# rsinghlab/GNN-Tumor-Seg

Hardware: AMD Instinct MI355X
Metric: supervoxel-graphs/sec training, 7xSAGE-pool-256, 15k-node graphs (higher is better)
Workload: dtype f32; 1 GPU; C2: 7xGraphSAGE-pool-256 (8 SAGEConv), fwd+weighted-CE+bwd+AdamW, 4 x 15000-node/86350-edge lattice graphs per GPU, 4-chan feat, fp32; global_batch=4, nodes_per_batch=60000, edges_per_batch=345400, parallelism=dp1

## Files before the change

### gnn-tumor-seg_amd/csrc/gts_gemm.hip

```cpp
#include "gts_gemm_tiles.h"
#include "gts_gemm_panel.h"
#include "gts_gemm_wgrad.h"
#include "gts_gemm_small.h"

namespace gts {
namespace {

template <bool AKC, bool BKC>
int pick_plain_variant(const GemmArgs& p) {
  int variant = BKC ? g_fwd_variant : g_igrad_variant;
  if (p.rb <= 128 && variant < 9) return 0;
  const bool row_count_invariant = variant == -2;
  if (variant < 0) {
    const int64_t cols = (p.rb + 255) / 256;
    const int64_t big_tiles = static_cast<int64_t>((p.ra + 255) / 256) * cols;
    variant = big_tiles >= 192 ? 8 : 3;
    if constexpr (AKC && BKC) {
      const int h = panel_rows_for(p.ra, cols);
      const int64_t panels = static_cast<int64_t>((p.ra + h - 1) / h) * cols;
      const int64_t rows256 = (big_tiles + 255) / 256 * 256, rows_panel = (panels + 255) / 256 * h;
      if (variant == 8 && rows_panel < rows256 && !row_count_invariant) variant = 10;
      if (variant == 3 && panels >= 192 && panels <= 256 && !row_count_invariant) variant = 10;
    }
  }
// ... 319 lines not shown
  r.splits = splits;
  int jobs = 0;
  for (int q = 0; q < n_problems; ++q, ++jobs) {
    r.slabs[jobs] = workspace + static_cast<size_t>(q) * splits * n * k;
    r.out[jobs] = gw[q], r.n4[jobs] = static_cast<int>(n * k / 4);
  }
  for (int q = 0; q < n_problems && any_bias; ++q) {
    if (!gb[q]) continue;
    r.slabs[jobs] = p.colsum + static_cast<size_t>(q) * splits * n;
    r.out[jobs] = gb[q], r.n4[jobs] = static_cast<int>(n / 4);
    ++jobs;
  }
  reduce_slabs_kernel<<<dim3(static_cast<unsigned>((n * k / 4 + 63) / 64), jobs), kBlock, 0, st>>>(r);
  return launch_status();
}
```

### gnn-tumor-seg_amd/csrc/gts_gemm_wgrad.h

```cpp
#pragma once
#include <type_traits>

#include "gts_gemm_tiles.h"

namespace gts {
namespace {

typedef float v2f __attribute__((ext_vector_type(2)));

template <int O0, int O1>
__device__ __forceinline__ v2f lds_read2st64(unsigned addr) {
  static_assert(O0 >= 0 && O1 <= 255, "ds_read2st64_b32 offsets are 8 bits");
  v2f r;
  asm volatile("ds_read2st64_b32 %0, %1 offset0:%2 offset1:%3" : "=v"(r) : "v"(addr), "n"(O0), "n"(O1));
  return r;
}

template <class Probe = NoProbe>
__global__ __launch_bounds__(1024, 4) void wgrad_stream_kernel(const GemmArgs p) {
  constexpr int BM = 256, BN = 256, WM = 4, WN = 4, WTM = 64, WTN = 64, TM = 2, TN = 2;
  constexpr int kPlane = kBK * BM;
  static_assert(BM == BN && kPlane * 4 == 128 * 256, "image I of an operand sits 128 offset units above image 0");
  __shared__ float lds[4 * kPlane];
  const int lane = threadIdx.x & 63, wave = __builtin_amdgcn_readfirstlane(threadIdx.x >> 6);
// ... 158 lines not shown
#pragma unroll 8
    for (int s = grp; s < p.splits; s += 4) acc += src[static_cast<size_t>(s) * n4];
  }
  part[grp][col] = acc;
  __syncthreads();
  if (grp == 0 && i < n4) {
    const v4f total = (part[0][col] + part[1][col]) + (part[2][col] + part[3][col]);
    reinterpret_cast<v4f*>(out)[i] = total;
  }
}

constexpr int kSkinnyMax = 9;
constexpr int kSkinnyChunks = 512;

template <int S>
__global__ __launch_bounds__(kBlock) void skinny_wgrad_kernel(const float* __restrict__ skinny, int s_cols,
                                                             const float* __restrict__ wide,
                                                             float* __restrict__ partial, int64_t m,
                                                             int w, int64_t rows_per_chunk) {
  __shared__ v4f red[kBlock];
  const int cols4 = w >> 2;
  const int lanes = cols4 >= kBlock ? 1 : kBlock / cols4;
  const int rl = cols4 >= kBlock ? 0 : threadIdx.x / cols4;
  const int64_t row0 = blockIdx.x * rows_per_chunk, row1 = min(m, row0 + rows_per_chunk);
  for (int q0 = 0; q0 < cols4; q0 += kBlock) {
    const int q = q0 + (cols4 >= kBlock ? threadIdx.x : threadIdx.x % cols4);
    const bool live = q < cols4 && rl < lanes;
    v4f acc[S];
#pragma unroll
    for (int i = 0; i < S; ++i) acc[i] = v4f{0.f, 0.f, 0.f, 0.f};
    if (live) {
#pragma unroll 4
      for (int64_t row = row0 + rl; row < row1; row += lanes) {
        const v4f f = *reinterpret_cast<const v4f*>(wide + static_cast<size_t>(row) * w + 4 * q);
#pragma unroll
// ... 3 lines not shown
#pragma unroll
    for (int i = 0; i < S; ++i) {
      v4f total = acc[i];
      if (lanes > 1) {
        __syncthreads();
        red[threadIdx.x] = acc[i];
        __syncthreads();
        if (rl == 0 && live) {
          for (int l = 1; l < lanes; ++l) total += red[l * cols4 + q];
        }
      }
      if (rl == 0 && live)
        *reinterpret_cast<v4f*>(partial + (static_cast<size_t>(blockIdx.x) * S + i) * w + 4 * q) = total;
    }
  }
}

__global__ __launch_bounds__(kBlock) void skinny_sum_kernel(const float* __restrict__ partial,
                                                           float* __restrict__ dst0,
                                                           float* __restrict__ dst1, int rows, int s_cols,
                                                           int w, int chunks, int transposed) {
  __shared__ float part[16][16];
  const int o = threadIdx.x & 15, lane = threadIdx.x >> 4;
  const int idx = blockIdx.x * 16 + o;
  const int total_out = rows * w;
  float acc = 0.f;
  if (idx < total_out) {
#pragma unroll 8
    for (int c = lane; c < chunks; c += 16) acc += partial[static_cast<size_t>(c) * total_out + idx];
  }
  part[lane][o] = acc;
  __syncthreads();
  if (lane != 0 || idx >= total_out) return;
  float sum = part[0][o];
#pragma unroll
  for (int l = 1; l < 16; ++l) sum += part[l][o];
  const int i = idx / w, j = idx - i * w;
  if (i < s_cols)
    dst0[transposed ? j * s_cols + i : i * w + j] = sum;
  else if (dst1 != nullptr)
    dst1[j] = sum;
}

inline int64_t skinny_workspace_floats(int64_t m, int64_t n, int64_t k) {
// ... 101 lines not shown
```

### gnn-tumor-seg_amd/csrc/gts_project.hip

```cpp
#include "gts_rows.h"

namespace gts {
namespace {

template <typename RowT>
__device__ __forceinline__ void store_row(RowT* dst, const RowT& v, int nt) {
  if (!nt) {
    *dst = v;
    return;
  }
  if constexpr (sizeof(RowT) == 16) {
    typedef unsigned u4 __attribute__((ext_vector_type(4)));
    __builtin_nontemporal_store(*reinterpret_cast<const u4*>(&v), reinterpret_cast<u4*>(dst));
  } else if constexpr (sizeof(RowT) == 8) {
    typedef unsigned u2 __attribute__((ext_vector_type(2)));
    __builtin_nontemporal_store(*reinterpret_cast<const u2*>(&v), reinterpret_cast<u2*>(dst));
  } else {
    __builtin_nontemporal_store(v, dst);
  }
}

constexpr int kVoxPerLane = 8;
constexpr int kVoxPerWave = kWave * kVoxPerLane;
constexpr int kVoxPerBlock = kVoxPerWave * kWavesPerBlock;
// ... 134 lines not shown
inline void launch_project_argmax(const int16_t* svs, const float* logits, const int16_t* relabel,
                                  int16_t* out, int64_t n_vox, int n_rows, int n_classes,
                                  uint8_t* occ, int dx, int dy, int dz, hipStream_t st) {
  const unsigned grid = stream_grid(n_vox);
  if (n_classes == 4 && (reinterpret_cast<uintptr_t>(logits) & 15) == 0)
    project_argmax_kernel<4><<<grid, kBlock, 0, st>>>(svs, logits, relabel, out, n_vox, n_rows, 4,
                                                      occ, dx, dy, dz);
  else
    project_argmax_kernel<0><<<grid, kBlock, 0, st>>>(svs, logits, relabel, out, n_vox, n_rows,
                                                      n_classes, occ, dx, dy, dz);
}

}
}

extern "C" int32_t gts_abi_version(void) { return 29; }

extern "C" const char* gts_error_string(int32_t code) {
  switch (code) {
    case GTS_OK: return "ok";
    case GTS_ERR_NULL: return "gts: required pointer is NULL";
    case GTS_ERR_SHAPE: return "gts: unsupported or inconsistent shape";
    case GTS_ERR_ARGKIND: return "gts: unsupported arg_bytes/row_bytes/mode";
    default: return code > 0 ? hipGetErrorString(static_cast<hipError_t>(code)) : "gts: unknown error";
  }
}

extern "C" int32_t gts_project_rows_i16(const int16_t* svs, const void* table,
                                        const void* bg_row, void* out, int64_t n_vox,
                                        int64_t n_rows, int32_t row_bytes, void* stream) {
  using namespace gts;
// ... 62 lines not shown
```

### gnn-tumor-seg_amd/csrc/gts_stack.hip

```cpp
#include <algorithm>
#include <vector>

#include "gts_gemm_args.h"

namespace {

constexpr int kMaxLayers = 64;

inline int64_t align256(int64_t bytes) { return (bytes + 255) & ~255LL; }

inline bool bad_stack(int64_t n_rows, const int64_t* widths, int32_t n_layers) {
  if (!widths || n_layers < 1 || n_layers > kMaxLayers || n_rows < 0 || n_rows >= (1LL << 31)) return true;
  for (int i = 0; i <= n_layers; ++i)
    if (widths[i] <= 0 || widths[i] % 4 != 0 || widths[i] >= (1 << 20)) return true;
  return false;
}

struct FwdPlan {
  int64_t m[kMaxLayers], arg[kMaxLayers], out[kMaxLayers], bits[kMaxLayers];
  int64_t p[2];
  int64_t wp[kMaxLayers][3];
  int64_t counters;
  int64_t total;
};
// ... 24 lines not shown
  p.total = at;
  return p;
}

inline bool chainable(int64_t n, int64_t k0, int64_t k1, int64_t n2) {
  return n % 4 == 0 && k0 % 4 == 0 && k1 % 4 == 0 && n <= 256 && n2 <= 256;
}

inline bool turns(int64_t rows, int64_t cols) { return cols >= 128 && rows % 4 == 0 && cols % 4 == 0; }

struct BwdPlan {
  int64_t wt[kMaxLayers][3];
  int64_t wtp[kMaxLayers][3];
  int64_t g[kMaxLayers], gp[kMaxLayers];
  int64_t gm[2];
  int64_t workspace, workspace_bytes;
  int64_t counters;
  int64_t total;
};

struct ByShape {
  struct Group {
    int64_t rows, cols;
    std::vector<const float*> in[2];
    std::vector<float*> out[2];
    int count() const { return static_cast<int>(in[0].size()); }
  };
  std::vector<Group> groups;
  void add(int64_t rows, int64_t cols, const float* in0, const float* in1, float* out0, float* out1) {
    auto it = std::find_if(groups.begin(), groups.end(), [&](const Group& c) { return c.rows == rows && c.cols == cols; });
// ... 6 lines not shown
inline int64_t weight_rows(const int64_t* w, int i, int q) { return q == 0 ? w[i] : w[i + 1]; }

inline BwdPlan plan_backward(int64_t n, const int64_t* w, int n_layers) {
  BwdPlan p{};
  int64_t at = 0, widest = 0;
  auto take = [&](int64_t bytes) { const int64_t o = at; at += align256(bytes); return o; };
  ByShape wgrads;
  for (int i = 0; i < n_layers; ++i) {
    const int64_t fin = w[i];
    widest = std::max(widest, fin);
    for (int q = 0; q < 3; ++q) p.wt[i][q] = turns(weight_rows(w, i, q), fin) ? take(4 * weight_rows(w, i, q) * fin) : -1;
    for (int q = 0; q < 3; ++q)
      p.wtp[i][q] = p.wt[i][q] >= 0 ? take(4 * gts_packed_weight_floats(fin, weight_rows(w, i, q))) : -1;
    p.g[i] = i > 0 ? take(4 * n * fin) : -1;
    p.gp[i] = take(4 * n * fin);
    for (int q = 0; q < 3; ++q) wgrads.add(weight_rows(w, i, q), fin, nullptr, nullptr, nullptr, nullptr);
  }
  p.gm[0] = take(4 * n * widest);
  p.gm[1] = take(4 * n * widest);
  int64_t ws = 0;
  if (n > 0)
    for (const auto& grp : wgrads.groups)
      for (int first = 0; first < grp.count(); first += gts::kMaxProblems)
        ws = std::max(ws, gts_linear_bwd_weight_workspace(n, grp.rows, grp.cols, std::min(gts::kMaxProblems, grp.count() - first)));
  p.workspace_bytes = ws;
  p.workspace = take(ws);
  p.counters = take(4 * GTS_CLUSTER_COUNTER_WORDS);
  p.total = at;
  return p;
}

// ... 150 lines not shown
  auto wt = [&](int i, int q) -> const float* { return plan.wt[i][q] >= 0 ? f32(plan.wt[i][q]) : nullptr; };
  auto wtp = [&](int i, int q) -> const float* { return plan.wtp[i][q] >= 0 ? f32(plan.wtp[i][q]) : nullptr; };

  auto igrad = [&](const float* g0, const float* w0, const float* w0t, int64_t n0, const float* g1, const float* w1,
                   const float* w1t, int64_t n1, const float* relu_mask, const uint64_t* relu_bits, float* gin,
                   int64_t k, const float* w0tp, const float* w1tp) -> int32_t {
    if (w0t != nullptr && (g1 == nullptr || w1t != nullptr)) {
      const float* packed[2] = {w0tp, g1 ? w1tp : nullptr};
      return gts_linear_bwd_input_t_f32(g0, w0t, g1, g1 ? w1t : nullptr, relu_mask, relu_mask ? relu_bits : nullptr, gin,
                                        n_rows, k, n0, g1 ? n1 : 0, packed, stream);
    }
    return gts_linear_bwd_input_f32(g0, w0, g1, g1 ? w1 : nullptr, relu_mask, gin, n_rows, k, n0, g1 ? n1 : 0, stream);
  };

  ByShape wgrads;

  const float* g = gout;
  const float* gm = nullptr;
  int cur = 0;
  for (int i = n_layers - 1; i >= 0; --i) {
    const float* w_pool = params[5 * i];
    const float* w_self = params[5 * i + 2];
    const float* w_neigh = params[5 * i + 3];
    const int64_t fin = widths[i], fout = widths[i + 1];
    const float* h = input_of(i);
    const float* m = act(fwd.m[i]);
    const void* arg = acts + fwd.arg[i];
    if (gm == nullptr) {
      float* buf = f32(plan.gm[cur]);
      GTS_TRY(igrad(g, w_neigh, wt(i, 2), fout, nullptr, nullptr, nullptr, 0, nullptr, nullptr, buf, fin, wtp(i, 2), nullptr));
      gm = buf;
    }
    float* gp = f32(plan.gp[i]);
    if (sched_rec != nullptr && fin == 256 && arg_bytes == 1 && n_rows * 1024 < (1LL << 32)) {
      GTS_TRY(gts_spmm_max_bwd_cluster_f32(sched_rec, sched_clusters, sched_rows, sched_srcs, sched_loc_words, gm, arg, 1, gp,
                                           n_rows, fin, counters, stream));
    } else {
      GTS_TRY(gts_spmm_max_bwd_f32(t_indptr, t_indices, t_slot, gm, arg, arg_bytes, nullptr, gp, n_rows, fin, stream));
    }
    gm = nullptr;
    wgrads.add(fin, fin, gp, h, grads[5 * i], grads[5 * i + 1]);
    wgrads.add(fout, fin, g, h, grads[5 * i + 2], grads[5 * i + 4]);
    wgrads.add(fout, fin, g, m, grads[5 * i + 3], nullptr);
    if (i > 0) {
      const int64_t below_in = widths[i - 1];
      const uint64_t* hbits = fwd.bits[i - 1] >= 0 ? reinterpret_cast<const uint64_t*>(acts + fwd.bits[i - 1]) : nullptr;
      float* g_next = f32(plan.g[i]);
      const float* below_t = wt(i - 1, 2);
      if (wt(i, 1) && wt(i, 0) && below_t && chainable(fin, fout, fin, below_in)) {
        float* gm_next = f32(plan.gm[cur ^ 1]);
        const float* packed[3] = {wtp(i, 1), wtp(i, 0), wtp(i - 1, 2)};
        GTS_TRY(gts_linear_bwd_input_chain_t_f32(g, wt(i, 1), gp, wt(i, 0), h, hbits, g_next, below_t, gm_next, n_rows, fin,
                                                 fout, fin, below_in, packed, stream));
        gm = gm_next, cur ^= 1;
      } else {
        GTS_TRY(igrad(g, w_self, wt(i, 1), fout, gp, w_pool, wt(i, 0), fin, h, hbits, g_next, fin, wtp(i, 1), wtp(i, 0)));
      }
      g = g_next;
    } else if (gx != nullptr) {
      GTS_TRY(igrad(g, w_self, wt(i, 1), fout, gp, w_pool, wt(i, 0), fin, nullptr, nullptr, gx, fin, wtp(i, 1), wtp(i, 0)));
    }
  }
  for (const auto& grp : wgrads.groups)
    for (int first = 0; first < grp.count(); first += gts::kMaxProblems)
      GTS_TRY(gts_linear_bwd_weight_f32(grp.in[0].data() + first, grp.in[1].data() + first, grp.out[0].data() + first,
                                        grp.out[1].data() + first, std::min(gts::kMaxProblems, grp.count() - first),
                                        f32(plan.workspace), plan.workspace_bytes, n_rows, grp.rows, grp.cols, stream));
  return GTS_OK;
}
```

### gnn-tumor-seg_amd/gts/_lib.py

```python
import ctypes
import os
import re

_HERE = os.path.dirname(os.path.abspath(__file__))
LIB_PATH = os.environ.get("GTS_LIB_PATH") or os.path.join(_HERE, "libgts_hip.so")
HEADER_PATH = os.path.join(os.path.dirname(os.path.dirname(_HERE)), "include", "gts_hip.h")
ABI_VERSION = 29

_p = ctypes.c_void_p
_i32 = ctypes.c_int32
_i64 = ctypes.c_int64
_f32 = ctypes.c_float
_f64 = ctypes.c_double

SIGNATURES = {
    "gts_abi_version": [],
    "gts_error_string": [_i32],
    "gts_spmm_max_fwd_f32": [_p, _p, _p, _p, _p, _i32, _i32, _i64, _i64, _p],
    "gts_spmm_max_bwd_f32": [_p, _p, _p, _p, _p, _i32, _p, _p, _i64, _i64, _p],
    "gts_cluster_record_words": [_i32, _i32, _i32, _i32],
    "gts_cluster_schedule": [_p, _p, _p, _p, _p, _i64, _i32, _i32, _i32, _p, _i64, _p, _p, _p],
    "gts_cluster_lds_bytes": [_i32, _i32, _i32, _i32],
    "gts_cluster_uses_counters": [_i64, _i32, _i32, _i32, _i32],
    "gts_spmm_max_fwd_cluster_f32": [_p, _i64, _i32, _i32, _i32, _p, _p, _p, _i32, _i32, _i64, _i64, _p, _p],
# ... 29 lines not shown
    "gts_relu_bits_bytes": [_i64, _i64],
    "gts_relu_bits_pay": [_i64, _i64],
    "gts_linear_bwd_input_f32": [_p, _p, _p, _p, _p, _p, _i64, _i64, _i64, _i64, _p],
    "gts_linear_bwd_input_t_f32": [_p, _p, _p, _p, _p, _p, _p, _i64, _i64, _i64, _i64, _p, _p],
    "gts_linear_bwd_input_t_act_workspace": [_i64, _i64],
    "gts_linear_bwd_input_t_act_f32": [_p, _p, _p, _p, _p, _i32, _p, _p, _p, _i64, _i64, _i64, _i64, _i64, _p, _p],
    "gts_transpose_batch_f32": [_p, _p, _i32, _i64, _i64, _p],
    "gts_packed_weight_floats": [_i64, _i64],
    "gts_pack_weights_f32": [_p, _p, _p, _i32, _i64, _i64, _i32, _p],
    "gts_gat_fc_scores_workspace": [_i64, _i64, _i64],
    "gts_gat_fc_scores_f32": [_p, _p, _p, _p, _p, _p, _p, _p, _i64, _i64, _i64, _i64, _i64, _p, _p],
    "gts_linear_fwd_chain_f32": [_p, _p, _p, _p, _p, _p, _p, _p, _p, _i64, _i64, _i64, _i64, _i32, _i64, _i32, _p, _p, _p],
    "gts_linear_bwd_input_chain_t_f32": [_p, _p, _p, _p, _p, _p, _p, _p, _p, _i64, _i64, _i64, _i64, _i64, _p, _p],
    "gts_linear_bwd_weight_workspace": [_i64, _i64, _i64, _i32],
    "gts_linear_bwd_weight_f32": [_p, _p, _p, _p, _i32, _p, _i64, _i64, _i64, _i64, _p],
    "gts_sage_pool_stack_fwd_arena": [_i64, _p, _i32, _i32, _i32, _i32, _p],
    "gts_sage_pool_stack_fwd_f32": [_p, _p, _p, _i64, _i32, _i32, _i32, _p, _p, _i64, _p, _i32, _i32, _i32, _i32, _p, _i64, _p],
    "gts_sage_pool_stack_bwd_scratch": [_i64, _p, _i32, _i32],
    "gts_sage_pool_stack_bwd_f32": [_p, _p, _p, _p, _i64, _i32, _i32, _i32, _p, _p, _p, _i64, _p, _i32, _i32, _i32, _p, _p, _p,
                                    _p, _i64, _p],
    "gts_set_option": [_i32, _i32],
    "gts_get_option": [_i32],
    "gts_weighted_ce_workspace": [_i64],
    "gts_weighted_ce_f32": [_p, _p, _p, _p, _p, _i64, _p, _i64, _i64, _p],
    "gts_dice_ce_workspace": [_i64, _i32],
    "gts_dice_ce_fwd_f32": [_p, _p, _p, _p, _i32, _f64, _f64, _f64, _p, _p, _i64, _i64, _i64, _p],
    "gts_dice_ce_bwd_f32": [_p, _p, _p, _p, _i32, _f64, _f64, _f64, _p, _p, _p, _i64, _i64, _p],
    "gts_collate_plan": [_p, _i32, _i64, _p, _i32, _p],
    "gts_collate_batch": [_p, _i32, _i64, _p, _i32, _p, _i64, _i32, _p],
    "gts_gg_gaussian_f64": [_p, _p, _p, _p, _i32, _f64, _i64, _i64, _i64, _i64, _p],
# ... 28 lines not shown
    "gts_intake_select_workspace": [],
    "gts_intake_order_stats": [_p, _i32, _i64, _i64, _i64, _p, _i64, _p, _i64, _p, _i64, _i64, _i64, _p, _p, _i64, _p],
    "gts_intake_standardize": [_p, _i32, _i64, _i64, _i64, _p, _i64, _p, _i64, _p, _i64, _p, _p, _p],
    "gts_dataset_stats_workspace": [_i64, _i64, _i64],
    "gts_dataset_stats_mask": [_p, _i32, _p, _i64, _i64, _i64, _p, _p, _i64, _p],
    "gts_dataset_stats_order_stats": [_p, _i32, _i64, _i64, _i64, _i64, _i64, _i64, _p, _p, _i64, _p],
    "gts_dataset_stats_moments": [_p, _i32, _i64, _i64, _i64, _i64, _p, _p, _p, _i64, _p],
    "gts_conform_gather": [_p, _i32, _i64, _i64, _i64, _i64, _i32, _i32, _i32, _i64, _i64, _i64, _p, _p, _p, _i32, _p, _p],
}
_RESTYPE = {"gts_error_string": ctypes.c_char_p, "gts_linear_bwd_weight_workspace": _i64,
            "gts_weighted_ce_workspace": _i64, "gts_gat_reduce_workspace": _i64,
            "gts_dice_ce_workspace": _i64,
            "gts_label_confusion_workspace": _i64, "gts_gat_fc_scores_workspace": _i64,
            "gts_relu_bits_bytes": _i64, "gts_cluster_record_words": _i64, "gts_sage_pool_stack_fwd_arena": _i64, "gts_sage_pool_stack_bwd_scratch": _i64, "gts_cluster_lds_bytes": _i64,
            "gts_linear_bwd_input_t_act_workspace": _i64, "gts_gat_cluster_workspace": _i64,
            "gts_packed_weight_floats": _i64, "gts_gg_sv_stats_workspace": _i64, "gts_gg_touching_workspace": _i64,
            "gts_conv3d_fwd_workspace": _i64, "gts_conv3d_bwd_data_workspace": _i64,
            "gts_conv3d_bwd_weight_workspace": _i64, "gts_hd95_workspace": _i64,
            "gts_intake_select_workspace": _i64, "gts_dataset_stats_workspace": _i64,
            "gts_components_workspace": _i64, "gts_lesionwise_workspace": _i64, "gts_lesionwise_table_ints": _i64}

COLLATE_MAX_SCHEDULES = 6


class CollateMember(ctypes.Structure):
    _fields_ = [("n_nodes", _i64), ("n_edges", _i64),
                ("indptr", _p), ("indices", _p), ("t_indptr", _p), ("t_indices", _p), ("t_slot", _p), ("t_pos", _p),
                ("features", _p), ("labels", _p), ("feat_bytes", _i32), ("label_bytes", _i32),
                ("sched_rec", _p * COLLATE_MAX_SCHEDULES), ("sched_clusters", _i64 * COLLATE_MAX_SCHEDULES),
                ("sched_loc_words", _i32 * COLLATE_MAX_SCHEDULES)]

# ... 80 lines not shown
```

### gnn-tumor-seg_amd/gts/dense.py

```python
import torch
import torch.nn.functional as F

from . import _lib
from ._lib import check, current_stream, ptr, require_device

GEMM_TIMER = None


class row_count_invariant:

    _depth = 0
    _saved = -1
    _lock = __import__("threading").Lock()

    def __enter__(self):
        with row_count_invariant._lock:
            if row_count_invariant._depth == 0:
                lib = _lib.load()
                row_count_invariant._saved = int(lib.gts_get_option(1))
                check(lib.gts_set_option(1, -2), "gts_set_option")
            row_count_invariant._depth += 1
        return self

    def __exit__(self, *exc):
# ... 342 lines not shown
                                          ptr(ws), ws.numel() * 4, m, n_p, k_p, current_stream()),
            "gts_linear_bwd_weight_f32"))
    out = []
    for gw, gb in zip(gws, gbs):
        if (n_p, k_p) != (n, k):
            gw = gw[:n, :k].contiguous()
            gb = gb[:n].contiguous() if gb is not None else None
        out.append((gw, gb))
    return out


def linear_bwd_weight(g, a, want_bias_grad=False):
    return linear_bwd_weight_multi([(g, a, want_bias_grad)])[0]


def relu_bwd(g, out):
    return g * (out > 0)


class _Linear(torch.autograd.Function):

    @staticmethod
    def forward(ctx, x, w, bias):
        ctx.save_for_backward(x, w)
        ctx.has_bias = bias is not None
        return linear_fwd(x, w, bias=bias)

    @staticmethod
    def backward(ctx, gy):
        x, w = ctx.saved_tensors
# ... 11 lines not shown
```

### gnn-tumor-seg_amd/gts/nn.py

```python
import os

import torch
import torch.nn as nn
import torch.nn.functional as F

from . import dense, ops


class GraphError(RuntimeError):
    """Counterpart of dgl.DGLError for the checks the layers make."""


def _is_relu(fn):
    return fn in (F.relu, torch.relu, torch.nn.functional.relu)


class _SagePoolLayer(torch.autograd.Function):

    @staticmethod
    def forward(ctx, g, h, w_pool, b_pool, w_self, w_neigh, bias, relu_out, need_bwd):
        h = h.contiguous()
        p = dense.linear_fwd(h, w_pool, bias=b_pool, relu=True)
        m, arg = ops.spmm_max_fwd(g, p, want_arg=need_bwd, relu_input=True)
        out = dense.linear_fwd(h, w_self, m, w_neigh, bias=bias, relu=relu_out)
# ... 163 lines not shown
        turned, turned_fragment = _pack_by_shape(
            [w for w in (params[5 * i + j] for i in range(n) for j in (0, 2, 3))
             if w.shape[1] >= 128 and w.shape[0] % 4 == 0 and w.shape[1] % 4 == 0], transposed=True, want_plain=True)

        def igrad(g0, w0, g1=None, w1=None, relu_mask=None, relu_bits=None):
            if id(w0) in turned and (w1 is None or id(w1) in turned) and g0.is_contiguous():
                return dense.linear_bwd_input_t(g0, turned[id(w0)], g1, turned[id(w1)] if w1 is not None else None,
                                                relu_mask=relu_mask, relu_bits=relu_bits,
                                                packed=(turned_fragment[id(w0)], turned_fragment[id(w1)] if w1 is not None else None))
            return dense.linear_bwd_input(g0, w0, g1, w1, relu_mask=relu_mask)

        def defer(grad_out, act, slot, bias_slot):
            key = (grad_out.shape[1], act.shape[1])
            deferred.setdefault(key, []).append((grad_out, act, bias_slot is not None, slot, bias_slot))

        gm = None
        for i in reversed(range(n)):
            h, m, arg, hbits = acts[4 * i:4 * i + 4]
            w_pool, _b_pool, w_self, w_neigh, _bias = params[5 * i:5 * i + 5]
            if gm is None:
                gm = igrad(g, w_neigh)
            gp = ops.spmm_max_bwd(ctx.g, gm, arg)
            gm = None
            defer(gp, h, 5 * i, 5 * i + 1)
            defer(g, h, 5 * i + 2, 5 * i + 4)
            defer(g, m, 5 * i + 3, None)
            if i > 0:
                below = params[5 * (i - 1) + 3]
                if all(id(w) in turned for w in (w_self, w_pool, below)) and _chainable(g, w_self.t(), gp, below.t()):
                    g, gm = dense.linear_bwd_input_chain_t(g, turned[id(w_self)], gp, turned[id(w_pool)], h,
                                                           turned[id(below)], relu_bits=hbits,
                                                           packed=(turned_fragment[id(w_self)], turned_fragment[id(w_pool)],
                                                                   turned_fragment[id(below)]))
                else:
                    g = igrad(g, w_self, gp, w_pool, relu_mask=h, relu_bits=hbits)
            elif ctx.needs_input_grad[1]:
                gx = igrad(g, w_self, gp, w_pool)
        for problems in deferred.values():
            results = dense.linear_bwd_weight_multi([(go, act, want) for go, act, want, _, _ in problems])
            for (gw, gb), (_, _, _, slot, bias_slot) in zip(results, problems):
                grads[slot] = gw
                if bias_slot is not None:
                    grads[bias_slot] = gb
        return (None, gx, None, *grads)


STACK_IN_ONE_CALL = os.environ.get("GTS_STACK_C", "1") != "0"


class GradSink:

    def __init__(self, params, extra=0):
        self.params = list(params)
        self.offsets, at = {}, 0
        for p in self.params:
            self.offsets[id(p)] = at
            at += p.numel()
        self.n, self.extra = at, int(extra)
# ... 394 lines not shown
```

### include/gts_hip.h

```cpp
#ifndef GTS_HIP_H
#define GTS_HIP_H

#include <stdint.h>

#ifdef __cplusplus
extern "C" {
#endif

#define GTS_OK 0
#define GTS_ERR_NULL (-1)
#define GTS_ERR_SHAPE (-2)
#define GTS_ERR_ARGKIND (-3)

int32_t gts_abi_version(void);
const char* gts_error_string(int32_t code);

int32_t gts_spmm_max_fwd_f32(const int32_t* indptr, const int32_t* indices, const float* x,
                             float* out, void* arg, int32_t arg_bytes, int32_t relu_input,
                             int64_t n_dst, int64_t n_feat, void* stream);

int32_t gts_spmm_max_bwd_f32(const int32_t* t_indptr, const int32_t* t_indices,
                             const int32_t* t_slot, const float* gout, const void* arg,
                             int32_t arg_bytes, const float* relu_src, float* gx,
                             int64_t n_src, int64_t n_feat, void* stream);
// ... 132 lines not shown
                                 float* out2, int64_t m, int64_t n, int64_t k0, int64_t k1, int32_t relu,
                                 int64_t n2, int32_t relu2, uint64_t* relu_bits, const float* const* packed,
                                 void* stream);
int32_t gts_linear_bwd_input_chain_t_f32(const float* g0, const float* w0t, const float* g1,
                                         const float* w1t, const float* relu_mask, const uint64_t* relu_bits,
                                         float* gin, const float* w2t, float* gin2, int64_t m, int64_t k,
                                         int64_t n0, int64_t n1, int64_t k2, const float* const* packed,
                                         void* stream);
int32_t gts_transpose_batch_f32(const float* const* src, float* const* dst, int32_t n_mats,
                                int64_t rows, int64_t cols, void* stream);
int64_t gts_linear_bwd_weight_workspace(int64_t m, int64_t n, int64_t k, int32_t n_problems);
int32_t gts_linear_bwd_weight_f32(const float* const* g, const float* const* a, float* const* gw,
                                  float* const* gb, int32_t n_problems, float* workspace,
                                  int64_t workspace_bytes, int64_t m, int64_t n, int64_t k,
                                  void* stream);

int64_t gts_sage_pool_stack_fwd_arena(int64_t n_rows, const int64_t* widths, int32_t n_layers, int32_t training,
                                      int32_t arg_bytes, int32_t relu_bits, int64_t* offsets);
int32_t gts_sage_pool_stack_fwd_f32(const int32_t* indptr, const int32_t* indices, const int32_t* sched_rec,
                                    int64_t sched_clusters, int32_t sched_rows, int32_t sched_srcs,
                                    int32_t sched_loc_words, const float* x, const float* const* params,
                                    int64_t n_rows, const int64_t* widths, int32_t n_layers, int32_t training,
                                    int32_t arg_bytes, int32_t relu_bits, void* arena, int64_t arena_bytes, void* stream);
int64_t gts_sage_pool_stack_bwd_scratch(int64_t n_rows, const int64_t* widths, int32_t n_layers, int32_t relu_bits);
int32_t gts_sage_pool_stack_bwd_f32(const int32_t* t_indptr, const int32_t* t_indices, const int32_t* t_slot,
                                    const int32_t* sched_rec, int64_t sched_clusters, int32_t sched_rows,
                                    int32_t sched_srcs, int32_t sched_loc_words, const float* gout, const float* x,
                                    const float* const* params, int64_t n_rows, const int64_t* widths,
                                    int32_t n_layers, int32_t arg_bytes, int32_t relu_bits, const void* fwd_arena,
                                    float* const* grads, float* gx, void* scratch, int64_t scratch_bytes,
// ... 176 lines not shown
```

Measured before the change: 955.8 graphs/s.

## Fuse narrow first/last SAGE layer backward into dedicated skinny kernels

Adds special backward paths for the narrow layers of the SAGE stack: the 4-channel input layer and the narrow output layer. For the first layer, one kernel fuses the input-gradient through w_neigh with the self/neigh weight-gradient partial sums and the bias sum. For the last layer, a skinny wgrad kernel also produces bias sums. Partials for all narrow layers are reduced at the end in a single batched sum-jobs kernel instead of going through the generic wide GEMM wgrad path. This cuts launches and wasted tile work on very skinny GEMMs, at the cost of extra workspace and more code paths.

```diff
diff --git a/gnn-tumor-seg_amd/csrc/gts_gemm.hip b/gnn-tumor-seg_amd/csrc/gts_gemm.hip
--- a/gnn-tumor-seg_amd/csrc/gts_gemm.hip
+++ b/gnn-tumor-seg_amd/csrc/gts_gemm.hip
@@ -357,3 +357,137 @@
   reduce_slabs_kernel<<<dim3(static_cast<unsigned>((n * k / 4 + 63) / 64), jobs), kBlock, 0, st>>>(r);
   return launch_status();
 }
+
+namespace gts {
+namespace {
+
+inline int narrow_kind(int64_t n, int64_t k) {
+  if (n <= 0 || k <= 0 || !aligned4(n) || !aligned4(k) || skinny_workspace_floats(1, n, k) == 0) return 0;
+  if (k < n) return (k == 4 || k == 8) && (n == 64 || n == 128 || n == 256) && g_igrad_variant <= 1 ? 1 : 0;
+  return n == 4 || n == 8 ? 2 : 0;
+}
+
+struct NarrowBlock {
+  int64_t first, second, sums, total;
+};
+inline NarrowBlock narrow_block(int kind, int64_t n, int64_t k) {
+  NarrowBlock b{};
+  if (kind == 1) b.second = kSkinnyChunks * (k + 1) * n, b.total = b.second + kSkinnyChunks * k * n;
+  if (kind == 2) b.second = kSkinnyChunks * n * k, b.sums = 2 * b.second, b.total = b.sums + kSkinnyChunks * n;
+  return b;
+}
+
+inline bool bad_narrow_rows(int64_t m) { return m < 0 || m >= (1LL << 31); }
+
+}
+}
+
+extern "C" int32_t gts_narrow_bwd_kind(int64_t n, int64_t k) { return gts::narrow_kind(n, k); }
+
+extern "C" int64_t gts_narrow_bwd_partial_floats(int64_t n, int64_t k) {
+  return gts::narrow_block(gts::narrow_kind(n, k), n, k).total;
+}
+
+extern "C" int32_t gts_narrow_bwd_first_f32(const float* g, const float* w_neigh, const float* x, const float* mact, float* gm,
+                                            float* partial, int32_t want_bias, int64_t m, int64_t n, int64_t k, void* stream) {
+  using namespace gts;
+  if (!g || !w_neigh || !x || !mact || !gm || !partial) return GTS_ERR_NULL;
+  if (bad_narrow_rows(m) || narrow_kind(n, k) != 1) return GTS_ERR_SHAPE;
+  if (m == 0) return GTS_OK;
+  hipStream_t st = static_cast<hipStream_t>(stream);
+  const NarrowBlock b = narrow_block(1, n, k);
+  const int64_t rpc = (m + kSkinnyChunks - 1) / kSkinnyChunks;
+  const int chunks = static_cast<int>((m + rpc - 1) / rpc), w = static_cast<int>(n);
+  float* px = partial;
+  float* pm = partial + b.second;
+  if (k == 4) {
+    if (want_bias) narrow_first_kernel<4, true><<<chunks, kBlock, 0, st>>>(g, w_neigh, x, mact, gm, px, pm, m, w, rpc);
+    else narrow_first_kernel<4, false><<<chunks, kBlock, 0, st>>>(g, w_neigh, x, mact, gm, px, pm, m, w, rpc);
+  } else {
+    if (want_bias) narrow_first_kernel<8, true><<<chunks, kBlock, 0, st>>>(g, w_neigh, x, mact, gm, px, pm, m, w, rpc);
+    else narrow_first_kernel<8, false><<<chunks, kBlock, 0, st>>>(g, w_neigh, x, mact, gm, px, pm, m, w, rpc);
+  }
+  return launch_status();
+}
+
+extern "C" int32_t gts_narrow_bwd_last_f32(const float* g, const float* h, const float* mact, float* partial, int32_t want_bias,
+                                           int64_t m, int64_t n, int64_t k, void* stream) {
+  using namespace gts;
+  if (!g || !h || !mact || !partial) return GTS_ERR_NULL;
+  if (bad_narrow_rows(m) || k >= (1 << 20) || narrow_kind(n, k) != 2) return GTS_ERR_SHAPE;
+  if (m == 0) return GTS_OK;
+  hipStream_t st = static_cast<hipStream_t>(stream);
+  const NarrowBlock b = narrow_block(2, n, k);
+  const int64_t rpc = (m + kSkinnyChunks - 1) / kSkinnyChunks;
+  const int chunks = static_cast<int>((m + rpc - 1) / rpc), s = static_cast<int>(n), w = static_cast<int>(k);
+  float* ph = partial;
+  float* pm = partial + b.second;
+  float* sums = partial + b.sums;
+  if (n == 4) {
+    if (want_bias) skinny_wgrad_sums_kernel<4><<<chunks, kBlock, 0, st>>>(g, s, h, ph, sums, m, w, rpc);
+    else skinny_wgrad_kernel<4><<<chunks, kBlock, 0, st>>>(g, s, h, ph, m, w, rpc);
+    skinny_wgrad_kernel<4><<<chunks, kBlock, 0, st>>>(g, s, mact, pm, m, w, rpc);
+  } else {
+    if (want_bias) skinny_wgrad_sums_kernel<8><<<chunks, kBlock, 0, st>>>(g, s, h, ph, sums, m, w, rpc);
+    else skinny_wgrad_kernel<8><<<chunks, kBlock, 0, st>>>(g, s, h, ph, m, w, rpc);
+    skinny_wgrad_kernel<8><<<chunks, kBlock, 0, st>>>(g, s, mact, pm, m, w, rpc);
+  }
+  return launch_status();
+}
+
+extern "C" int32_t gts_narrow_bwd_finish_f32(const float* const* partial, float* const* gw_self, float* const* gw_neigh,
+                                             float* const* gb, const int64_t* n, const int64_t* k, int32_t n_layers, int64_t m,
+                                             void* stream) {
+  using namespace gts;
+  if (!partial || !gw_self || !gw_neigh || !n || !k) return GTS_ERR_NULL;
+  if (n_layers < 1 || n_layers > kMaxProblems) return GTS_ERR_ARGKIND;
+  if (bad_narrow_rows(m)) return GTS_ERR_SHAPE;
+  for (int i = 0; i < n_layers; ++i) {
+    if (!partial[i] || !gw_self[i] || !gw_neigh[i]) return GTS_ERR_NULL;
+    if (narrow_kind(n[i], k[i]) == 0) return GTS_ERR_SHAPE;
+  }
+  hipStream_t st = static_cast<hipStream_t>(stream);
+  if (m == 0) {
+    for (int i = 0; i < n_layers; ++i) {
+      if (hipMemsetAsync(gw_self[i], 0, 4 * n[i] * k[i], st) != hipSuccess) return launch_status();
+      if (hipMemsetAsync(gw_neigh[i], 0, 4 * n[i] * k[i], st) != hipSuccess) return launch_status();
+      if (gb && gb[i] && hipMemsetAsync(gb[i], 0, 4 * n[i], st) != hipSuccess) return launch_status();
+    }
+    return GTS_OK;
+  }
+  const int64_t rpc = (m + kSkinnyChunks - 1) / kSkinnyChunks;
+  SkinnySumJobs jobs{};
+  jobs.chunks = static_cast<int>((m + rpc - 1) / rpc);
+  int count = 0, widest = 0;
+  auto flush = [&]() -> int {
+    if (count == 0) return GTS_OK;
+    skinny_sum_jobs_kernel<<<dim3(static_cast<unsigned>((widest + 15) / 16), count), kBlock, 0, st>>>(jobs);
+    count = 0, widest = 0;
+    return launch_status();
+  };
+  auto add = [&](const float* part, float* dst0, float* dst1, int rows, int s_cols, int w, int transposed) {
+    jobs.partial[count] = part, jobs.dst0[count] = dst0, jobs.dst1[count] = dst1;
+    jobs.rows[count] = rows, jobs.s_cols[count] = s_cols, jobs.w[count] = w, jobs.transposed[count] = transposed;
+    widest = rows * w > widest ? rows * w : widest;
+    ++count;
+  };
+  for (int i = 0; i < n_layers; ++i) {
+    if (count + 3 > kMaxSumJobs) {
+      const int rc = flush();
+      if (rc != GTS_OK) return rc;
+    }
+    const int kind = narrow_kind(n[i], k[i]);
+    const NarrowBlock b = narrow_block(kind, n[i], k[i]);
+    float* bias = gb ? gb[i] : nullptr;
+    const int ni = static_cast<int>(n[i]), ki = static_cast<int>(k[i]);
+    if (kind == 1) {
+      add(partial[i], gw_self[i], bias, ki + (bias ? 1 : 0), ki, ni, 1);
+      add(partial[i] + b.second, gw_neigh[i], nullptr, ki, ki, ni, 1);
+    } else {
+      add(partial[i], gw_self[i], nullptr, ni, ni, ki, 0);
+      add(partial[i] + b.second, gw_neigh[i], nullptr, ni, ni, ki, 0);
+      if (bias) add(partial[i] + b.sums, nullptr, bias, 1, 0, ni, 0);
+    }
+  }
+  return flush();
+}
diff --git a/gnn-tumor-seg_amd/csrc/gts_gemm_wgrad.h b/gnn-tumor-seg_amd/csrc/gts_gemm_wgrad.h
--- a/gnn-tumor-seg_amd/csrc/gts_gemm_wgrad.h
+++ b/gnn-tumor-seg_amd/csrc/gts_gemm_wgrad.h
@@ -196,11 +196,9 @@
 constexpr int kSkinnyChunks = 512;
 
 template <int S>
-__global__ __launch_bounds__(kBlock) void skinny_wgrad_kernel(const float* __restrict__ skinny, int s_cols,
-                                                             const float* __restrict__ wide,
-                                                             float* __restrict__ partial, int64_t m,
-                                                             int w, int64_t rows_per_chunk) {
-  __shared__ v4f red[kBlock];
+__device__ __forceinline__ void skinny_wgrad_chunk(const float* __restrict__ skinny, int s_cols,
+                                                   const float* __restrict__ wide, float* __restrict__ partial,
+                                                   int64_t m, int w, int64_t rows_per_chunk, v4f* red) {
   const int cols4 = w >> 2;
   const int lanes = cols4 >= kBlock ? 1 : kBlock / cols4;
   const int rl = cols4 >= kBlock ? 0 : threadIdx.x / cols4;
@@ -234,6 +232,101 @@
         *reinterpret_cast<v4f*>(partial + (static_cast<size_t>(blockIdx.x) * S + i) * w + 4 * q) = total;
     }
   }
+}
+
+template <int S>
+__global__ __launch_bounds__(kBlock) void skinny_wgrad_kernel(const float* __restrict__ skinny, int s_cols,
+                                                             const float* __restrict__ wide,
+                                                             float* __restrict__ partial, int64_t m,
+                                                             int w, int64_t rows_per_chunk) {
+  __shared__ v4f red[kBlock];
+  skinny_wgrad_chunk<S>(skinny, s_cols, wide, partial, m, w, rows_per_chunk, red);
+}
+
+template <int S>
+__global__ __launch_bounds__(kBlock) void skinny_wgrad_sums_kernel(const float* __restrict__ skinny, int s_cols,
+                                                                  const float* __restrict__ wide,
+                                                                  float* __restrict__ partial, float* __restrict__ sums,
+                                                                  int64_t m, int w, int64_t rows_per_chunk) {
+  __shared__ v4f red[kBlock];
+  skinny_wgrad_chunk<S>(skinny, s_cols, wide, partial, m, w, rows_per_chunk, red);
+  skinny_wgrad_chunk<1>(nullptr, 0, skinny, sums, m, s_cols, rows_per_chunk, red);
+}
+
+template <int S, bool ONES>
+__global__ __launch_bounds__(kBlock) void narrow_first_kernel(const float* __restrict__ g, const float* __restrict__ w_neigh,
+                                                             const float* __restrict__ x, const float* __restrict__ mact,
+                                                             float* __restrict__ gm, float* __restrict__ part_x,
+                                                             float* __restrict__ part_m, int64_t m, int w,
+                                                             int64_t rows_per_chunk) {
+  constexpr int RX = S + (ONES ? 1 : 0);
+  __shared__ v4f red[kBlock];
+  const int cols4 = w >> 2;
+  const int lanes = kBlock / cols4;
+  const int rl = threadIdx.x / cols4, q = threadIdx.x % cols4;
+  const int64_t row0 = blockIdx.x * rows_per_chunk, row1 = min(m, row0 + rows_per_chunk);
+  v4f wn[S];
+#pragma unroll
+  for (int e = 0; e < 4; ++e)
+#pragma unroll
+    for (int n4 = 0; n4 < S; n4 += 4) {
+      const v4f t = *reinterpret_cast<const v4f*>(w_neigh + static_cast<size_t>(4 * q + e) * S + n4);
+#pragma unroll
+      for (int j = 0; j < 4; ++j) wn[n4 + j][e] = t[j];
+    }
+  v4f ax[RX], am[S];
+#pragma unroll
+  for (int i = 0; i < RX; ++i) ax[i] = v4f{0.f, 0.f, 0.f, 0.f};
+#pragma unroll
+  for (int i = 0; i < S; ++i) am[i] = v4f{0.f, 0.f, 0.f, 0.f};
+#pragma unroll 4
+  for (int64_t row = row0 + rl; row < row1; row += lanes) {
+    const v4f f = *reinterpret_cast<const v4f*>(g + static_cast<size_t>(row) * w + 4 * q);
+    float xs[S], ms[S];
+#pragma unroll
+    for (int n4 = 0; n4 < S; n4 += 4) {
+      const v4f tx = *reinterpret_cast<const v4f*>(x + row * S + n4), tm = *reinterpret_cast<const v4f*>(mact + row * S + n4);
+#pragma unroll
+      for (int j = 0; j < 4; ++j) xs[n4 + j] = tx[j], ms[n4 + j] = tm[j];
+    }
+#pragma unroll
+    for (int i = 0; i < RX; ++i) ax[i] += (i < S ? xs[i < S ? i : 0] : 1.0f) * f;
+#pragma unroll
+    for (int i = 0; i < S; ++i) am[i] += ms[i] * f;
+    float dot[S];
+#pragma unroll
+    for (int n = 0; n < S; ++n) {
+      dot[n] = 0.f;
+#pragma unroll
+      for (int e = 0; e < 4; ++e) dot[n] = __builtin_fmaf(f[e], wn[n][e], dot[n]);
+    }
+#pragma unroll
+    for (int n = 0; n < S; ++n) {
+      for (int o = 32; o >= cols4; o >>= 1) dot[n] += 0.f;
+      for (int o = cols4 >> 1; o > 0; o >>= 1) dot[n] += __shfl_xor(dot[n], o, kWave);
+    }
+    if (q == 0) {
+#pragma unroll
+      for (int n4 = 0; n4 < S; n4 += 4)
+        *reinterpret_cast<v4f*>(gm + row * S + n4) = v4f{dot[n4], dot[n4 + 1], dot[n4 + 2], dot[n4 + 3]};
+    }
+  }
+  auto combine = [&](const v4f mine, float* out_row) __attribute__((always_inline)) {
+    v4f total = mine;
+    if (lanes > 1) {
+      __syncthreads();
+      red[threadIdx.x] = mine;
+      __syncthreads();
+      if (rl == 0) {
+        for (int l = 1; l < lanes; ++l) total += red[l * cols4 + q];
+      }
+    }
+    if (rl == 0) *reinterpret_cast<v4f*>(out_row + 4 * q) = total;
+  };
+#pragma unroll
+  for (int i = 0; i < RX; ++i) combine(ax[i], part_x + (static_cast<size_t>(blockIdx.x) * RX + i) * w);
+#pragma unroll
+  for (int i = 0; i < S; ++i) combine(am[i], part_m + (static_cast<size_t>(blockIdx.x) * S + i) * w);
 }
 
 __global__ __launch_bounds__(kBlock) void skinny_sum_kernel(const float* __restrict__ partial,
@@ -248,6 +341,47 @@
   if (idx < total_out) {
 #pragma unroll 8
     for (int c = lane; c < chunks; c += 16) acc += partial[static_cast<size_t>(c) * total_out + idx];
+  }
+  part[lane][o] = acc;
+  __syncthreads();
+  if (lane != 0 || idx >= total_out) return;
+  float sum = part[0][o];
+#pragma unroll
+  for (int l = 1; l < 16; ++l) sum += part[l][o];
+  const int i = idx / w, j = idx - i * w;
+  if (i < s_cols)
+    dst0[transposed ? j * s_cols + i : i * w + j] = sum;
+  else if (dst1 != nullptr)
+    dst1[j] = sum;
+}
+
+constexpr int kMaxSumJobs = 16;
+struct SkinnySumJobs {
+  const float* partial[kMaxSumJobs];
+  float* dst0[kMaxSumJobs];
+  float* dst1[kMaxSumJobs];
+  int rows[kMaxSumJobs], s_cols[kMaxSumJobs], w[kMaxSumJobs], transposed[kMaxSumJobs];
+  int chunks;
+};
+
+__global__ __launch_bounds__(kBlock) void skinny_sum_jobs_kernel(const SkinnySumJobs p) {
+  __shared__ float part[16][16];
+  const int job = blockIdx.y;
+  const float* partial = kernarg_entry<const float*>(offsetof(SkinnySumJobs, partial), job);
+  float* dst0 = kernarg_entry<float*>(offsetof(SkinnySumJobs, dst0), job);
+  float* dst1 = kernarg_entry<float*>(offsetof(SkinnySumJobs, dst1), job);
+  const int rows = kernarg_entry<int>(offsetof(SkinnySumJobs, rows), job);
+  const int s_cols = kernarg_entry<int>(offsetof(SkinnySumJobs, s_cols), job);
+  const int w = kernarg_entry<int>(offsetof(SkinnySumJobs, w), job);
+  const int transposed = kernarg_entry<int>(offsetof(SkinnySumJobs, transposed), job);
+  const int total_out = rows * w;
+  if (static_cast<int>(blockIdx.x) * 16 >= total_out) return;
+  const int o = threadIdx.x & 15, lane = threadIdx.x >> 4;
+  const int idx = blockIdx.x * 16 + o;
+  float acc = 0.f;
+  if (idx < total_out) {
+#pragma unroll 8
+    for (int c = lane; c < p.chunks; c += 16) acc += partial[static_cast<size_t>(c) * total_out + idx];
   }
   part[lane][o] = acc;
   __syncthreads();
diff --git a/gnn-tumor-seg_amd/csrc/gts_project.hip b/gnn-tumor-seg_amd/csrc/gts_project.hip
--- a/gnn-tumor-seg_amd/csrc/gts_project.hip
+++ b/gnn-tumor-seg_amd/csrc/gts_project.hip
@@ -172,7 +172,7 @@
 }
 }
 
-extern "C" int32_t gts_abi_version(void) { return 29; }
+extern "C" int32_t gts_abi_version(void) { return 30; }
 
 extern "C" const char* gts_error_string(int32_t code) {
   switch (code) {
diff --git a/gnn-tumor-seg_amd/csrc/gts_stack.hip b/gnn-tumor-seg_amd/csrc/gts_stack.hip
--- a/gnn-tumor-seg_amd/csrc/gts_stack.hip
+++ b/gnn-tumor-seg_amd/csrc/gts_stack.hip
@@ -62,6 +62,7 @@
   int64_t wtp[kMaxLayers][3];
   int64_t g[kMaxLayers], gp[kMaxLayers];
   int64_t gm[2];
+  int64_t narrow[kMaxLayers];
   int64_t workspace, workspace_bytes;
   int64_t counters;
   int64_t total;
@@ -98,7 +99,9 @@
       p.wtp[i][q] = p.wt[i][q] >= 0 ? take(4 * gts_packed_weight_floats(fin, weight_rows(w, i, q))) : -1;
     p.g[i] = i > 0 ? take(4 * n * fin) : -1;
     p.gp[i] = take(4 * n * fin);
-    for (int q = 0; q < 3; ++q) wgrads.add(weight_rows(w, i, q), fin, nullptr, nullptr, nullptr, nullptr);
+    const bool narrow = gts_narrow_bwd_kind(w[i + 1], fin) != 0;
+    p.narrow[i] = narrow ? take(4 * gts_narrow_bwd_partial_floats(w[i + 1], fin)) : -1;
+    for (int q = 0; q < (narrow ? 1 : 3); ++q) wgrads.add(weight_rows(w, i, q), fin, nullptr, nullptr, nullptr, nullptr);
   }
   p.gm[0] = take(4 * n * widest);
   p.gm[1] = take(4 * n * widest);
@@ -279,6 +282,13 @@
   };
 
   ByShape wgrads;
+  std::vector<const float*> narrow_partial;
+  std::vector<float*> narrow_self, narrow_neigh, narrow_bias;
+  std::vector<int64_t> narrow_n, narrow_k;
+  auto finish_later = [&](int i) {
+    narrow_partial.push_back(f32(plan.narrow[i])), narrow_n.push_back(widths[i + 1]), narrow_k.push_back(widths[i]);
+    narrow_self.push_back(grads[5 * i + 2]), narrow_neigh.push_back(grads[5 * i + 3]), narrow_bias.push_back(grads[5 * i + 4]);
+  };
 
   const float* g = gout;
   const float* gm = nullptr;
@@ -291,7 +301,12 @@
     const float* h = input_of(i);
     const float* m = act(fwd.m[i]);
     const void* arg = acts + fwd.arg[i];
-    if (gm == nullptr) {
+    const int narrow = gts_narrow_bwd_kind(fout, fin);
+    if (narrow == 1) {
+      float* buf = f32(plan.gm[cur]);
+      GTS_TRY(gts_narrow_bwd_first_f32(g, w_neigh, h, m, buf, f32(plan.narrow[i]), 1, n_rows, fout, fin, stream));
+      gm = buf;
+    } else if (gm == nullptr) {
       float* buf = f32(plan.gm[cur]);
       GTS_TRY(igrad(g, w_neigh, wt(i, 2), fout, nullptr, nullptr, nullptr, 0, nullptr, nullptr, buf, fin, wtp(i, 2), nullptr));
       gm = buf;
@@ -305,8 +320,13 @@
     }
     gm = nullptr;
     wgrads.add(fin, fin, gp, h, grads[5 * i], grads[5 * i + 1]);
-    wgrads.add(fout, fin, g, h, grads[5 * i + 2], grads[5 * i + 4]);
-    wgrads.add(fout, fin, g, m, grads[5 * i + 3], nullptr);
+    if (narrow == 0) {
+      wgrads.add(fout, fin, g, h, grads[5 * i + 2], grads[5 * i + 4]);
+      wgrads.add(fout, fin, g, m, grads[5 * i + 3], nullptr);
+    } else {
+      if (narrow == 2) GTS_TRY(gts_narrow_bwd_last_f32(g, h, m, f32(plan.narrow[i]), 1, n_rows, fout, fin, stream));
+      finish_later(i);
+    }
     if (i > 0) {
       const int64_t below_in = widths[i - 1];
       const uint64_t* hbits = fwd.bits[i - 1] >= 0 ? reinterpret_cast<const uint64_t*>(acts + fwd.bits[i - 1]) : nullptr;
@@ -331,5 +351,10 @@
       GTS_TRY(gts_linear_bwd_weight_f32(grp.in[0].data() + first, grp.in[1].data() + first, grp.out[0].data() + first,
                                         grp.out[1].data() + first, std::min(gts::kMaxProblems, grp.count() - first),
                                         f32(plan.workspace), plan.workspace_bytes, n_rows, grp.rows, grp.cols, stream));
+  for (size_t first = 0; first < narrow_partial.size(); first += gts::kMaxProblems)
+    GTS_TRY(gts_narrow_bwd_finish_f32(narrow_partial.data() + first, narrow_self.data() + first, narrow_neigh.data() + first,
+                                      narrow_bias.data() + first, narrow_n.data() + first, narrow_k.data() + first,
+                                      static_cast<int32_t>(std::min<size_t>(gts::kMaxProblems, narrow_partial.size() - first)),
+                                      n_rows, stream));
   return GTS_OK;
 }
diff --git a/gnn-tumor-seg_amd/gts/_lib.py b/gnn-tumor-seg_amd/gts/_lib.py
--- a/gnn-tumor-seg_amd/gts/_lib.py
+++ b/gnn-tumor-seg_amd/gts/_lib.py
@@ -5,7 +5,7 @@
 _HERE = os.path.dirname(os.path.abspath(__file__))
 LIB_PATH = os.environ.get("GTS_LIB_PATH") or os.path.join(_HERE, "libgts_hip.so")
 HEADER_PATH = os.path.join(os.path.dirname(os.path.dirname(_HERE)), "include", "gts_hip.h")
-ABI_VERSION = 29
+ABI_VERSION = 30
 
 _p = ctypes.c_void_p
 _i32 = ctypes.c_int32
@@ -67,6 +67,11 @@
     "gts_linear_bwd_input_chain_t_f32": [_p, _p, _p, _p, _p, _p, _p, _p, _p, _i64, _i64, _i64, _i64, _i64, _p, _p],
     "gts_linear_bwd_weight_workspace": [_i64, _i64, _i64, _i32],
     "gts_linear_bwd_weight_f32": [_p, _p, _p, _p, _i32, _p, _i64, _i64, _i64, _i64, _p],
+    "gts_narrow_bwd_kind": [_i64, _i64],
+    "gts_narrow_bwd_partial_floats": [_i64, _i64],
+    "gts_narrow_bwd_first_f32": [_p, _p, _p, _p, _p, _p, _i32, _i64, _i64, _i64, _p],
+    "gts_narrow_bwd_last_f32": [_p, _p, _p, _p, _i32, _i64, _i64, _i64, _p],
+    "gts_narrow_bwd_finish_f32": [_p, _p, _p, _p, _p, _p, _i32, _i64, _p],
     "gts_sage_pool_stack_fwd_arena": [_i64, _p, _i32, _i32, _i32, _i32, _p],
     "gts_sage_pool_stack_fwd_f32": [_p, _p, _p, _i64, _i32, _i32, _i32, _p, _p, _i64, _p, _i32, _i32, _i32, _i32, _p, _i64, _p],
     "gts_sage_pool_stack_bwd_scratch": [_i64, _p, _i32, _i32],
@@ -125,7 +130,7 @@
             "gts_label_confusion_workspace": _i64, "gts_gat_fc_scores_workspace": _i64,
             "gts_relu_bits_bytes": _i64, "gts_cluster_record_words": _i64, "gts_sage_pool_stack_fwd_arena": _i64, "gts_sage_pool_stack_bwd_scratch": _i64, "gts_cluster_lds_bytes": _i64,
             "gts_linear_bwd_input_t_act_workspace": _i64, "gts_gat_cluster_workspace": _i64,
-            "gts_packed_weight_floats": _i64, "gts_gg_sv_stats_workspace": _i64, "gts_gg_touching_workspace": _i64,
+            "gts_packed_weight_floats": _i64, "gts_narrow_bwd_partial_floats": _i64, "gts_gg_sv_stats_workspace": _i64, "gts_gg_touching_workspace": _i64,
             "gts_conv3d_fwd_workspace": _i64, "gts_conv3d_bwd_data_workspace": _i64,
             "gts_conv3d_bwd_weight_workspace": _i64, "gts_hd95_workspace": _i64,
             "gts_intake_select_workspace": _i64, "gts_dataset_stats_workspace": _i64,
diff --git a/gnn-tumor-seg_amd/gts/dense.py b/gnn-tumor-seg_amd/gts/dense.py
--- a/gnn-tumor-seg_amd/gts/dense.py
+++ b/gnn-tumor-seg_amd/gts/dense.py
@@ -380,6 +380,64 @@
     return linear_bwd_weight_multi([(g, a, want_bias_grad)])[0]
 
 
+def narrow_bwd_kind(n, k):
+    return int(_lib.load().gts_narrow_bwd_kind(n, k))
+
+
+def _narrow_partial(n, k, dev):
+    return torch.empty(int(_lib.load().gts_narrow_bwd_partial_floats(n, k)), dtype=torch.float32, device=dev)
+
+
+def narrow_bwd_first(g, w_neigh, x, mact, want_bias=True):
+    m, n, k = g.shape[0], g.shape[1], x.shape[1]
+    _same(tuple(_mat(w_neigh, "w_neigh").shape), (n, k), "w_neigh vs g, x")
+    _same(tuple(mact.shape), (m, k), "mact vs x")
+    _same(x.shape[0], m, "rows of g / x")
+    g, w_neigh, x, mact = _dense(g, w_neigh, x, mact)
+    dev = _chk(g, w_neigh, x, mact)
+    gm = torch.empty((m, k), dtype=torch.float32, device=dev)
+    partial = _narrow_partial(n, k, dev)
+    if m == 0:
+        return gm, partial
+    _timed("wgrad", 6.0 * m * n * k, lambda: check(
+        _lib.load().gts_narrow_bwd_first_f32(ptr(g), ptr(w_neigh), ptr(x), ptr(mact), ptr(gm), ptr(partial),
+                                             1 if want_bias else 0, m, n, k, current_stream()), "gts_narrow_bwd_first_f32"))
+    return gm, partial
+
+
+def narrow_bwd_last(g, h, mact, want_bias=True):
+    m, n, k = g.shape[0], g.shape[1], h.shape[1]
+    _same(tuple(_mat(h, "h").shape), (m, k), "h vs g")
+    _same(tuple(_mat(mact, "mact").shape), (m, k), "mact vs h")
+    g, h, mact = _dense(g, h, mact)
+    dev = _chk(g, h, mact)
+    partial = _narrow_partial(n, k, dev)
+    if m == 0:
+        return partial
+    _timed("wgrad", 4.0 * m * n * k, lambda: check(
+        _lib.load().gts_narrow_bwd_last_f32(ptr(g), ptr(h), ptr(mact), ptr(partial), 1 if want_bias else 0, m, n, k,
+                                            current_stream()), "gts_narrow_bwd_last_f32"))
+    return partial
+
+
+def narrow_bwd_finish(layers, m):
+    import ctypes
+
+    if len(layers) > MAX_WGRAD_PROBLEMS:
+        return narrow_bwd_finish(layers[:MAX_WGRAD_PROBLEMS], m) + narrow_bwd_finish(layers[MAX_WGRAD_PROBLEMS:], m)
+    dev = _chk(*[p for p, _, _, _ in layers])
+    out = [(torch.empty((n, k), dtype=torch.float32, device=dev), torch.empty((n, k), dtype=torch.float32, device=dev),
+            torch.empty(n, dtype=torch.float32, device=dev) if want else None) for _, n, k, want in layers]
+    q = len(layers)
+    arr, dims = ctypes.c_void_p * q, ctypes.c_int64 * q
+    _timed("wgrad", 0.0, lambda: check(
+        _lib.load().gts_narrow_bwd_finish_f32(arr(*[ptr(p) for p, _, _, _ in layers]), arr(*[ptr(o[0]) for o in out]),
+                                              arr(*[ptr(o[1]) for o in out]), arr(*[ptr(o[2]) for o in out]),
+                                              dims(*[n for _, n, _, _ in layers]), dims(*[k for _, _, k, _ in layers]), q, m,
+                                              current_stream()), "gts_narrow_bwd_finish_f32"))
+    return out
+
+
 def relu_bwd(g, out):
     return g * (out > 0)
 
diff --git a/gnn-tumor-seg_amd/gts/nn.py b/gnn-tumor-seg_amd/gts/nn.py
--- a/gnn-tumor-seg_amd/gts/nn.py
+++ b/gnn-tumor-seg_amd/gts/nn.py
@@ -201,17 +201,26 @@
             key = (grad_out.shape[1], act.shape[1])
             deferred.setdefault(key, []).append((grad_out, act, bias_slot is not None, slot, bias_slot))
 
+        narrow_layers = []
         gm = None
         for i in reversed(range(n)):
             h, m, arg, hbits = acts[4 * i:4 * i + 4]
             w_pool, _b_pool, w_self, w_neigh, _bias = params[5 * i:5 * i + 5]
-            if gm is None:
+            narrow = dense.narrow_bwd_kind(w_self.shape[0], w_self.shape[1])
+            if narrow == 1:
+                gm, partial = dense.narrow_bwd_first(g, w_neigh, h, m)
+            elif gm is None:
                 gm = igrad(g, w_neigh)
             gp = ops.spmm_max_bwd(ctx.g, gm, arg)
             gm = None
             defer(gp, h, 5 * i, 5 * i + 1)
-            defer(g, h, 5 * i + 2, 5 * i + 4)
-            defer(g, m, 5 * i + 3, None)
+            if narrow == 0:
+                defer(g, h, 5 * i + 2, 5 * i + 4)
+                defer(g, m, 5 * i + 3, None)
+            else:
+                if narrow == 2:
+                    partial = dense.narrow_bwd_last(g, h, m)
+                narrow_layers.append((partial, w_self.shape[0], w_self.shape[1], True, i))
             if i > 0:
                 below = params[5 * (i - 1) + 3]
                 if all(id(w) in turned for w in (w_self, w_pool, below)) and _chainable(g, w_self.t(), gp, below.t()):
@@ -229,6 +238,10 @@
                 grads[slot] = gw
                 if bias_slot is not None:
                     grads[bias_slot] = gb
+        if narrow_layers:
+            results = dense.narrow_bwd_finish([layer[:4] for layer in narrow_layers], gout.shape[0])
+            for (gw_self, gw_neigh, gb), (_, _, _, _, i) in zip(results, narrow_layers):
+                grads[5 * i + 2], grads[5 * i + 3], grads[5 * i + 4] = gw_self, gw_neigh, gb
         return (None, gx, None, *grads)
 
 
diff --git a/include/gts_hip.h b/include/gts_hip.h
--- a/include/gts_hip.h
+++ b/include/gts_hip.h
@@ -170,6 +170,15 @@
                                   float* const* gb, int32_t n_problems, float* workspace,
                                   int64_t workspace_bytes, int64_t m, int64_t n, int64_t k,
                                   void* stream);
+int32_t gts_narrow_bwd_kind(int64_t n, int64_t k);
+int64_t gts_narrow_bwd_partial_floats(int64_t n, int64_t k);
+int32_t gts_narrow_bwd_first_f32(const float* g, const float* w_neigh, const float* x, const float* mact, float* gm,
+                                 float* partial, int32_t want_bias, int64_t m, int64_t n, int64_t k, void* stream);
+int32_t gts_narrow_bwd_last_f32(const float* g, const float* h, const float* mact, float* partial, int32_t want_bias,
+                                int64_t m, int64_t n, int64_t k, void* stream);
+int32_t gts_narrow_bwd_finish_f32(const float* const* partial, float* const* gw_self, float* const* gw_neigh,
+                                  float* const* gb, const int64_t* n, const int64_t* k, int32_t n_layers, int64_t m,
+                                  void* stream);
 
 int64_t gts_sage_pool_stack_fwd_arena(int64_t n_rows, const int64_t* widths, int32_t n_layers, int32_t training,
                                       int32_t arg_bytes, int32_t relu_bits, int64_t* offsets);
```

After: 958.1 graphs/s (median of 3 runs). Within noise of the previous version (+0.2%).
